# paritytech/reed-solomon-novelpoly

Hardware: AMD Instinct MI355X
Metric: payload GiB/s (device-resident) encode+reconstruct, n=1024 shards, 1 MiB msgs (higher is better)
Workload: dtype u16; 1 GPU; BASELINE config 3: n_wanted=1024 k_wanted=342 (effective n=1024, k=256), 1048576 B payloads, batch 1024/GPU, encode + error locator + reconstruct with 342 random erasures per payload; n=1024, k=256, payload_bytes=1048576, batch_per_gpu=1024, global_batch=1024, erasures=342, parallelism=replicas x1 (no collective)

## Files before the change

### reed-solomon-novelpoly_amd/csrc/fast_common.hpp

```cpp
#pragma once
#include <type_traits>

#include "device_common.hpp"
#include "launchers.hpp"

namespace np {
namespace {

constexpr int kTile = 256;

#ifndef NP_EXP
#define NP_EXP 0
#endif
constexpr int kExp = NP_EXP;

__device__ __forceinline__ void stamp(uint64_t* dbg, int slot) {
  if constexpr ((kExp & 64) != 0 && (kExp & 128) != 0) {
    if ((threadIdx.x & 63u) == 0) dbg[32u * (threadIdx.x >> 6) + slot] = __builtin_amdgcn_s_memtime();
  } else if constexpr (kExp & 64) {
    if (threadIdx.x == 0) dbg[slot] = __builtin_amdgcn_s_memtime();
  }
}
constexpr int kPoolWords = 20;

// ... 955 lines not shown
    x = s;
    y = d;
  } else {
    const int32_t a = static_cast<int32_t>(x), b = static_cast<int32_t>(y);
    x = static_cast<uint32_t>(a + b);
    y = static_cast<uint32_t>(a - b);
  }
}
template <int N, int NT, bool MOD>
__device__ __forceinline__ void lds_wht(uint32_t* W) {
  const uint32_t tid = threadIdx.x;
  int b = 0;
#pragma unroll 1
  for (; (2 << b) < N; b += 2) {
    const uint32_t h = 1u << b;
    for (uint32_t q = tid; q < N / 4; q += NT) {
      const uint32_t i = ((q & ~(h - 1u)) << 2) | (q & (h - 1u));
      uint32_t x0 = W[i], x1 = W[i + h], x2 = W[i + 2 * h], x3 = W[i + 3 * h];
      wht_bfly<MOD>(x0, x1);
      wht_bfly<MOD>(x2, x3);
      wht_bfly<MOD>(x0, x2);
      wht_bfly<MOD>(x1, x3);
      W[i] = x0, W[i + h] = x1, W[i + 2 * h] = x2, W[i + 3 * h] = x3;
    }
    __syncthreads();
  }
  if ((1 << b) < N) {
    const uint32_t h = 1u << b;
    for (uint32_t q = tid; q < N / 2; q += NT) {
      const uint32_t i = ((q & ~(h - 1u)) << 1) | (q & (h - 1u));
      uint32_t x = W[i], y = W[i + h];
      wht_bfly<MOD>(x, y);
      W[i] = x, W[i + h] = y;
    }
    __syncthreads();
  }
}

template <int N, int NT>
__device__ __forceinline__ void fused_locator_core(const DevTables& T, uint32_t* W, uint16_t* E, const uint8_t* PR) {
  const uint32_t tid = threadIdx.x;
  lds_wht<N, NT, false>(W);
  const uint16_t* F = T.lw_fold + N;
  for (uint32_t v = tid; v < N; v += NT) {
    const int32_t x = static_cast<int32_t>(W[v]);
    const uint32_t m = x < 0 ? static_cast<uint32_t>(x + 65535) : static_cast<uint32_t>(x);
    W[v] = (m * static_cast<uint32_t>(F[v])) % 65535u;
  }
  __syncthreads();
  lds_wht<N, NT, true>(W);
  for (uint32_t v = tid; v < N; v += NT) *NP_BCHK(E + v, 2, kBkRecords) = T.exp[NP_ICHK(PR[v] ? W[v] : 65535u - W[v], 65536u)];
}

template <int N, int NT>
__device__ __forceinline__ void fused_locator_pools(const DevTables& T, uint32_t* W, const uint8_t* PR, uint8_t* dst) {
  const uint32_t tid = threadIdx.x;
  lds_wht<N, NT, false>(W);
  const uint16_t* F = T.lw_fold + N;
  for (uint32_t v = tid; v < N; v += NT) {
    const int32_t x = static_cast<int32_t>(W[v]);
    const uint32_t m = x < 0 ? static_cast<uint32_t>(x + 65535) : static_cast<uint32_t>(x);
    W[v] = (m * static_cast<uint32_t>(F[v])) % 65535u;
  }
  __syncthreads();
  lds_wht<N, NT, true>(W);
  for (uint32_t v = tid; v < N; v += NT) {
    const bool p = PR[v] != 0;
    const uint32_t e = T.exp[NP_ICHK(p ? W[v] : 65535u - W[v], 65536u)];
    const uint4* src = reinterpret_cast<const uint4*>((p ? T.in_pools : T.out_pools) + static_cast<size_t>(e) * kPoolWords);
    uint4* d = NP_BCHK(reinterpret_cast<uint4*>(dst + static_cast<size_t>(v) * 4 * kPoolWords), 4 * kPoolWords, kBkRecords);
    const uint4 a0 = src[0], a1 = src[1], a2 = src[2], a3 = src[3], a4 = src[4];
    d[0] = a0, d[1] = a1, d[2] = a2, d[3] = a3, d[4] = a4;
  }
}

template <int N, int NT>
__device__ __forceinline__ void fused_locator(const DevTables& T, const uint8_t* pres, uint32_t* W, uint16_t* E,
                                              uint8_t* PR) {
  const uint32_t tid = threadIdx.x;
  for (uint32_t v = tid; v < N; v += NT) {
    const uint8_t p = *NP_BCHK(pres + v, 1, kBkPresent);
    PR[v] = p;
    W[v] = p ? 0u : 1u;
  }
  __syncthreads();
  fused_locator_core<N, NT>(T, W, E, PR);
}

}
}
```

### reed-solomon-novelpoly_amd/csrc/kernels_fast.hip

```cpp
#include <algorithm>
#include <cstdlib>

#include "fast_common.hpp"

namespace np {
namespace {

constexpr int kEncMaxGen = 3;
__device__ __forceinline__ bool enc_tower(uint32_t index) {
  return __builtin_amdgcn_readfirstlane(gen_of(index)) <= static_cast<uint32_t>(kEncMaxGen);
}

constexpr int kEncPrio = 1, kEncPrioCq = 1;
constexpr int kRecPrioPremul = 2, kRecPrioCq = 3, kRecPrioHi = 2, kRecPrioFwdHi = 3, kRecPrioFwdCq = 2;

template <int K, int SH>
constexpr int kShiftGen = static_cast<int>(gen_of((SH == 23 ? 2 : SH) * K));

template <int K, int SH, typename HOOK = NoHiHook>
__device__ __forceinline__ void shift_hi(const DevTables& T, const uint32_t* vp, uint32_t index,
                                         const uint32_t (&ML)[16], const uint32_t (&MH)[16], uint32_t (&XL)[16],
                                         uint32_t (&XH)[16], uint32_t (&PL)[8], uint32_t (&PH)[8], HOOK hook = HOOK{}) {
#pragma unroll
  for (int q = 0; q < 16; ++q) {
// ... 554 lines not shown
__global__ __launch_bounds__(4 * K) __attribute__((amdgpu_waves_per_eu(4))) void k_encode_multi(EncLaunch L) {
#if defined(__HIP_DEVICE_COMPILE__)
  extern __shared__ __attribute__((aligned(16))) uint8_t smem[];
#if NP_BOUNDS_CHECK
  bounds_arm(bounds_of_enc(L.a));
#endif
  const uint32_t groups = (L.tiles + L.tpw - 1) / L.tpw;
  const TileRef tr = tile_of(blockIdx.x, groups, (L.a.batch & 7u) == 0);
  const uint32_t pb = tr.pb, tl0 = tr.tl * L.tpw;
  const uint32_t ntl = min(L.tpw, L.tiles - tl0);
  const uint64_t kp = reinterpret_cast<uint64_t>(__builtin_amdgcn_kernarg_segment_ptr());
  bool dma = false;
#pragma unroll 1
  for (uint32_t t = 0; t < ntl; ++t) {
    if (t > 0) __syncthreads();
    const enc_launch_ptr lp = reinterpret_cast<enc_launch_ptr>(fresh(kp));
    const DevTables T = lp->T;
    const EncodeArgs a = lp->a;
    const uint32_t pch0 = (tl0 + t - 1) * kTile;
    const bool stored16 = t > 0 && pch0 + kTile <= lp->nchunks &&
                          rows_vec_ok(a.shards, a.batch_stride, a.shard_len) &&
                          (min(a.n / K, (a.wanted_n + K - 1) / K) - 1) * K + 16 * 16 <= a.wanted_n &&
                          16 * a.shard_len < 0x7fffffffu;
    dma = encode_tile_multi<K>(T, a, smem, fresh(pb), fresh(tl0) + t, lp->nchunks, t == 0, dma, stored16,
                               t + 1 < ntl ? tl0 + t + 1 : ~0u);
  }
#endif
}

struct RecCtx {
  const DevTables& T;
  size_t shard_len;
  uint8_t* tile;
  const uint32_t* R;
  const uint8_t* sh;
  uint32_t* VP;
  uint32_t g, lane, tid, ncols;
  bool full;
  uint32_t cqb, hb;
  uint64_t* dbg;
  uint32_t occ;
};

template <int NQ>
__host__ __device__ constexpr int seg_of(int step) {
  return NQ == 8 ? 7 - step : NQ == 4 ? (step == 0 ? 2 : step == 1 ? 3 : 3 - step) : 1 - step;
}

__host__ __device__ constexpr uint32_t rec8_kappa(int q) {
  constexpr uint32_t k[8] = {1, 1, 3, 2, 12, 15, 10, 8};
  return k[q];
}

__device__ __forceinline__ uint32_t row_mask16(const uint8_t* pres, uint32_t row0, uint32_t lane) {
  const bool p = lane < 16u && *NP_BCHK(pres + (row0 + lane), 1, kBkPresent) != 0;
  return static_cast<uint32_t>(__ballot(p));
}

template <int CPOL>
__device__ __forceinline__ void issue_rows_c(uint2 (&raw)[16], const uint8_t* sh, size_t shard_len, uint32_t mask,
                                             uint32_t row0, const uint8_t* zeros, uint32_t lane, uint32_t ncols,
                                             bool full) {
  if (full) {
#pragma unroll
    for (int p = 0; p < 16; ++p) {
      if ((mask >> p) & 1u) NP_BNOTE(sh + static_cast<size_t>(row0 + p) * shard_len + 8u * lane, 8, kBkShards);
      const __amdgpu_buffer_rsrc_t r = buf_rsrc(sh + static_cast<size_t>(row0 + p) * shard_len, ((mask >> p) & 1u) ? 512u : 0u);
      const u32x2 v = __builtin_amdgcn_raw_buffer_load_b64(r, 8u * lane, 0, CPOL);
      raw[p] = make_uint2(v.x, v.y);
    }
  } else {
#pragma unroll
    for (int p = 0; p < 16; ++p) {
      const uint8_t* src = ((mask >> p) & 1u) ? sh + static_cast<size_t>(row0 + p) * shard_len : zeros;
      raw[p] = load4(src, lane, ncols, false);
    }
  }
}

__device__ __forceinline__ void issue_rows(uint2 (&raw)[16], const uint8_t* sh, size_t shard_len, uint32_t mask,
                                           uint32_t row0, const uint8_t* zeros, uint32_t lane, uint32_t ncols,
                                           bool full, bool reread = false) {
  if (!reread)
    issue_rows_c<2>(raw, sh, shard_len, mask, row0, zeros, lane, ncols, full);
  else
    issue_rows_c<0>(raw, sh, shard_len, mask, row0, zeros, lane, ncols, full);
}

template <int K>
__device__ __forceinline__ void copy_out_cq(uint8_t* out_tile, uint32_t lane, uint32_t g, const uint32_t (&L)[16],
                                            const uint32_t (&H)[16]) {
  uint2 d[4][4];
#pragma unroll
  for (int u = 0; u < 4; ++u) cq_to_blks(&L[4 * u], &H[4 * u], d[u]);
#pragma unroll
  for (int i = 0; i < 4; ++i) {
    uint8_t* o = NP_BCHK(out_tile + static_cast<size_t>(4u * lane + i) * 2 * K + 32u * g, 32, kBkOut);
    *reinterpret_cast<uint4*>(o) = make_uint4(d[0][i].x, d[0][i].y, d[1][i].x, d[1][i].y);
    *reinterpret_cast<uint4*>(o + 16) = make_uint4(d[2][i].x, d[2][i].y, d[3][i].x, d[3][i].y);
  }
}


template <int NQ>
constexpr bool kRowPrefetch = NQ <= 2;

template <int K, int NQ>
constexpr bool kRecResident =
    NQ > 1 &&
    Geo<K>::kTileBytes + NQ * 4u * Geo<K>::kVPWords <= 160u * 1024u * Geo<K>::kThreads / 1024u;
template <int K, int NQ>
__device__ __forceinline__ uint32_t vp_slot(int q, int step) {
  return kRecResident<K, NQ> ? static_cast<uint32_t>(q) : static_cast<uint32_t>(step & 1);
}

template <int K, int NQ>
constexpr int kRecMaxGen = static_cast<int>(gen_of(static_cast<uint32_t>((NQ - 1) * K)));

template <int K, int NQ>
__device__ __forceinline__ void stage_rec_tables(const DevTables& T, uint32_t* VP) {
  if constexpr (kRecResident<K, NQ>) {
#pragma unroll 1
    for (int q = 0; q < NQ; ++q)
      stage_vpools<K, Geo<K>::kThreads>(T, static_cast<uint32_t>(q) * K, VP + q * Geo<K>::kVPWords, true);
  } else {
    stage_vpools<K, Geo<K>::kThreads>(T, static_cast<uint32_t>(seg_of<NQ>(0)) * K, VP, true);
    stage_vpools<K, Geo<K>::kThreads>(T, static_cast<uint32_t>(seg_of<NQ>(1)) * K, VP + Geo<K>::kVPWords, true);
  }
}

template <int NQ>
__device__ __forceinline__ uint32_t seg_mask(const uint32_t (&msk)[NQ], int step) {
  if constexpr (NQ <= 2) return step == 0 ? msk[0] : msk[NQ - 1];
  uint64_t lo = 0, hi = 0;
#pragma unroll
  for (int i = 0; i < NQ; ++i) {
    const uint64_t v = static_cast<uint64_t>(msk[i] & 0xffffu);
    if (i < 4)
      lo |= v << (16 * i);
    else
      hi |= v << (16 * (i - 4));
  }
  const uint32_t sh = 16u * static_cast<uint32_t>(step & 3);
  return static_cast<uint32_t>(((step < 4 ? lo : hi) >> sh) & 0xffffu);
}

template <int K, int NQ>
constexpr bool kTilePrefetch = NQ == 4 && kMultiTile<K>;

template <int NQ>
constexpr bool kSkipEmpty = NQ == 8;

template <int K, int NQ, bool PRE0 = false>
__device__ __forceinline__ void rec_segments(const RecCtx& c, const uint32_t (&msk)[NQ], uint2 (&raw)[16],
                                             uint32_t (&AL)[16], uint32_t (&AH)[16], bool after_tile) {
  const DevTables& T = c.T;
  uint32_t XL[16], XH[16];
  auto fold = [&](int step, int q) __attribute__((always_inline)) {
    if (NQ == 8 && q != 0) {
      const uint32_t kq = uniform(rec8_kappa(q));
      if (kq == 1u) {
#pragma unroll
        for (int j = 0; j < 16; ++j) {
          AL[j] ^= XL[j];
          AH[j] ^= XH[j];
        }
      } else {
        uint32_t kp[20];
        pool_of<true>(T, kq, kp);
        const Mult pool = make_mult(kp);
        if (step == 0) {
#pragma unroll
          for (int j = 0; j < 16; ++j) qmul_sub_set(AL[j], AH[j], XL[j], XH[j], pool);
        } else {
#pragma unroll
          for (int j = 0; j < 16; ++j) qmul_sub(AL[j], AH[j], XL[j], XH[j], pool);
        }
      }
    } else if (step == 0) {
#pragma unroll
      for (int j = 0; j < 16; ++j) {
        AL[j] = XL[j];
        AH[j] = XH[j];
      }
    } else if (q == 0) {
      if (NQ == 2 || NQ == 8) {
#pragma unroll
        for (int j = 0; j < 16; ++j) {
          AL[j] ^= XL[j];
          AH[j] ^= XH[j];
        }
      }
      add_derivative<K>(AL, XL, c.tid % Geo<K>::R);
      add_derivative<K>(AH, XH, c.tid % Geo<K>::R);
    } else if (NQ == 4 && q == 3) {
      uint32_t beta[20];
      pool_of<true>(T, 2u, beta);
      const Mult pool = make_mult(beta);
#pragma unroll
      for (int j = 0; j < 16; ++j) {
        XL[j] ^= AL[j];
        XH[j] ^= AH[j];
        qmul_sub(AL[j], AH[j], XL[j], XH[j], pool);
      }
    } else {
#pragma unroll
      for (int j = 0; j < 16; ++j) {
        AL[j] ^= XL[j];
        AH[j] ^= XH[j];
      }
    }
  };
#pragma unroll 1
  for (int step = 0; step < NQ; ++step) {
    const int q = seg_of<NQ>(step);
    if (kSkipEmpty<NQ> && !((c.occ >> q) & 1u)) {
#pragma unroll
      for (int j = 0; j < 16; ++j) XL[j] = XH[j] = 0;
      if constexpr (!kRecResident<K, NQ>) {
        if (step > 0 && step + 1 < NQ) {
          __syncthreads();
          stage_vpools<K, Geo<K>::kThreads>(T, static_cast<uint32_t>(seg_of<NQ>(step + 1)) * K,
                                            c.VP + ((step + 1) & 1) * Geo<K>::kVPWords, true);
          __syncthreads();
        }
      }
    } else {
      const uint32_t index = uniform(static_cast<uint32_t>(q) * K);
      __builtin_amdgcn_sched_barrier(0);
      const uint32_t g = fresh(c.g);
      const uint8_t* sh = fresh(c.sh);
      const uint32_t* R = fresh(c.R);
      const size_t shard_len = fresh(c.shard_len);
      const uint32_t cqb = fresh_v(c.cqb), hb = fresh_v(c.hb);
      uint32_t m = uniform(seg_mask<NQ>(msk, step));
      if (!kRowPrefetch<NQ> && !(PRE0 && step == 0))
        issue_rows(raw, (kExp & 32) ? T.zeros : sh, (kExp & 32) ? 0 : shard_len, m, index + 16 * g, T.zeros, c.lane,
                   c.ncols, c.full, q == 0);
      stamp(c.dbg, 2 + 6 * step);
      __builtin_amdgcn_s_setprio(kRecPrioPremul);
      pipelined_rec<16>(
          [&](auto pc) __attribute__((always_inline)) {
            NP_BNOTE(reinterpret_cast<const uint8_t*>(R) + (index + 16 * g + decltype(pc)::value) * 4 * kPoolWords,
                     4 * kPoolWords, kBkRecords);
            return (cpool_t)(R) + (index + 16 * g + decltype(pc)::value) * kPoolWords;
          },
          [&](auto pc) __attribute__((always_inline)) { return ((m >> decltype(pc)::value) & 1u) != 0; },
          [&](auto pc, const Mult& pool) __attribute__((always_inline)) {
            constexpr int x = decltype(pc)::value;
            XL[x] = 0;
            XH[x] = 0;
            if ((m >> x) & 1u) {
              uint32_t l, h;
              blk_to_quad(raw[x], l, h);
              if constexpr (kExp & 16) {
                XL[x] = l;
                XH[x] = h;
// ... 286 lines not shown
#pragma unroll
          for (int e = 0; e < 8; ++e) o[e] = static_cast<uint8_t>((e < 4 ? v.x : v.y) >> (8 * (e & 3)));
        }
      }
    }
    stamp(dbg, 31);
  }
}

template <int K, int NQ, int SERVE>
__global__ __launch_bounds__(4 * K) __attribute__((amdgpu_waves_per_eu(4))) void k_reconstruct_fast(
    DevTables T, ReconstructArgs a, uint32_t nsyms, uint32_t tiles, uint32_t tpw) {
  constexpr int N = NQ * K;
  extern __shared__ __attribute__((aligned(16))) uint8_t smem[];
#if NP_BOUNDS_CHECK
  bounds_arm(bounds_of(a, T, prefix_stride_c(N, K)));
#endif
  const uint32_t groups = (tiles + tpw - 1) / tpw;
  const TileRef tr = tile_of(blockIdx.x, groups, (a.batch & 7u) == 0);
  const uint32_t pb = tr.pb, tl0 = tr.tl * tpw;
  const uint32_t ntl = min(tpw, tiles - tl0);
  const uint8_t* pres = a.present + static_cast<size_t>(pb) * N;
  const uint8_t* rec = NP_BCHK(a.prefix + static_cast<size_t>(pb) * prefix_stride_c(N, K), 2, kBkRecords);
  const int nq = uniform(rec[0]);
  const uint32_t occ = uniform(rec[1]);
  const uint32_t* rows = reinterpret_cast<const uint32_t*>(rec + prefix_pools_offset(N));
  if constexpr (kMultiTile<K>) {
    if constexpr (SERVE >= 4) {
      if (nq == SERVE) rec_tiles<K, SERVE>(T, a, pres, rows, smem, pb, tl0, ntl, nsyms, occ);
    } else if (nq == 1) {
      rec_tiles<K, 1>(T, a, pres, rows, smem, pb, tl0, ntl, nsyms, occ);
    } else if (NQ <= 4 && nq == 2) {
      rec_tiles<K, 2>(T, a, pres, rows, smem, pb, tl0, ntl, nsyms, occ);
    }
  } else {
    const uint32_t col0 = tl0 * kTile;
    const uint32_t ncols = min(static_cast<uint32_t>(kTile), nsyms - col0);
    const uint8_t* sh = a.shards + static_cast<size_t>(pb) * a.batch_stride + 2 * static_cast<size_t>(col0);
    const bool full =
        ncols == kTile && rows_vec_ok(a.shards, a.batch_stride, a.shard_len);
    uint64_t* dbg = (kExp & 64) ? reinterpret_cast<uint64_t*>(a.out + static_cast<size_t>(pb) * a.out_stride +
                                                               static_cast<size_t>(nsyms) * 2 * K + ((kExp & 128) ? 4096u : 256u) * tl0)
                                 : nullptr;
    if constexpr (SERVE >= 4) {
      if (nq == SERVE) rec_tile<K, SERVE>(T, a, sh, pres, rows, smem, pb, col0, ncols, full, dbg, occ);
    } else if (nq == 1) {
      rec_tile<K, 1>(T, a, sh, pres, rows, smem, pb, col0, ncols, full, dbg, occ);
    } else if (NQ <= 4 && nq == 2) {
      rec_tile<K, 2>(T, a, sh, pres, rows, smem, pb, col0, ncols, full, dbg, occ);
    }
  }
}

__device__ __forceinline__ void write_row_pools(const DevTables& T, const uint16_t* E, const uint8_t* PR,
                                                uint32_t rows, uint8_t* dst) {
  for (uint32_t v = threadIdx.x; v < rows; v += 256) {
    const uint32_t* pools = PR[v] ? T.in_pools : T.out_pools;
    const uint4* src = reinterpret_cast<const uint4*>(pools + static_cast<size_t>(NP_ICHK(*NP_BCHK(E + v, 2, kBkRecords), 65536u)) * kPoolWords);
    uint4* d = NP_BCHK(reinterpret_cast<uint4*>(dst + static_cast<size_t>(v) * 4 * kPoolWords), 4 * kPoolWords, kBkRecords);
    const uint4 a0 = src[0], a1 = src[1], a2 = src[2], a3 = src[3], a4 = src[4];
    d[0] = a0, d[1] = a1, d[2] = a2, d[3] = a3, d[4] = a4;
  }
}


template <int K, int N>
__device__ __forceinline__ void count_present(const uint8_t* pres, int& have1, int& have2, int& have) {
  have1 = have2 = have = 0;
  for (int r = 0; r < N; r += 256) {
    const int v = static_cast<int>(threadIdx.x) + r;
    const bool p = v < N && *NP_BCHK(pres + v, 1, kBkPresent) != 0;
    if (r < K) have1 += __syncthreads_count(v < K && p);
    if (r < 2 * K) have2 += __syncthreads_count(v < 2 * K && p);
    have += __syncthreads_count(p);
  }
}

template <int K, int N>
__device__ __forceinline__ uint32_t segment_occupancy(const uint8_t* pres) {
  uint32_t occ = 0;
#pragma unroll 1
  for (int q = 0; q < N / K; ++q) {
    int any = 0;
    for (int v = static_cast<int>(threadIdx.x); v < K; v += 256) any |= *NP_BCHK(pres + (q * K + v), 1, kBkPresent) != 0;
    if (__syncthreads_or(any)) occ |= 1u << q;
  }
  return occ;
}

__device__ __forceinline__ bool write_status(const ReconstructArgs& a, uint32_t pb, int have) {
  const bool ok = have >= static_cast<int>(a.k);
  if (threadIdx.x == 0 && a.status) {
    *NP_BCHK(a.status + 2 * pb, 4, kBkStatus) = ok ? 0u : kStatusNeedMoreShards;
    *NP_BCHK(a.status + 2 * pb + 1, 4, kBkStatus) = static_cast<uint32_t>(have);
  }
  return ok;
}

template <int N>
constexpr int kPrefixThreads = N >= 512 ? 512 : 256;

template <int K, int NQ, int NT = kPrefixThreads<NQ * K>>
__global__ __launch_bounds__(NT) void k_prefix_locator(DevTables T, ReconstructArgs a, uint8_t* out) {
  constexpr int N = NQ * K;
  __shared__ uint32_t W[N];
  __shared__ uint8_t PR[N];
  const uint32_t pb = blockIdx.x, tid = threadIdx.x;
#if NP_BOUNDS_CHECK
  {
    ReconstructArgs ab = a;
    ab.prefix = out;
    bounds_arm(bounds_of(ab, T, prefix_stride_c(N, K)));
  }
#endif
  const uint8_t* pres = a.present + static_cast<size_t>(pb) * N;
  uint8_t* rec = out + static_cast<size_t>(pb) * prefix_stride_c(N, K);
  __shared__ uint32_t acc[4];
  if (tid < 4) acc[tid] = 0;
  __syncthreads();
  {
    uint32_t c1 = 0, c2 = 0, c = 0, occ = 0;
    for (uint32_t v = tid; v < static_cast<uint32_t>(N); v += NT) {
      const uint8_t p = *NP_BCHK(pres + v, 1, kBkPresent);
      PR[v] = p;
      W[v] = p ? 0u : 1u;
      const uint32_t on = p ? 1u : 0u;
      c += on;
      c1 += v < static_cast<uint32_t>(K) ? on : 0u;
      c2 += v < 2u * K ? on : 0u;
      occ |= on << (v / K);
    }
#pragma unroll
    for (int o = 32; o > 0; o >>= 1) {
      c1 += __shfl_xor(c1, o);
      c2 += __shfl_xor(c2, o);
      c += __shfl_xor(c, o);
      occ |= __shfl_xor(occ, o);
    }
    if ((tid & 63u) == 0) {
      atomicAdd(&acc[0], c1);
      atomicAdd(&acc[1], c2);
      atomicAdd(&acc[2], c);
      atomicOr(&acc[3], occ);
    }
  }
  __syncthreads();
  const int have1 = static_cast<int>(acc[0]), have2 = static_cast<int>(acc[1]), have = static_cast<int>(acc[2]);
  const int nq = !write_status(a, pb, have) ? 0 : have1 == K ? 1 : (a.trusted && NQ == 4 && have2 >= K) ? 2 : NQ;
  if (tid == 0) *NP_BCHK(rec, 2, kBkRecords) = static_cast<uint8_t>(nq), *NP_BCHK(rec + 1, 1, kBkRecords) = static_cast<uint8_t>(acc[3]);
  if (nq <= 1) return;
  if (NQ == 4 && nq == 2) {
    fused_locator_pools<2 * K, NT>(T, W, PR, rec + prefix_pools_offset(N));
  } else {
    fused_locator_pools<N, NT>(T, W, PR, rec + prefix_pools_offset(N));
  }
}

template <int K, int NQ>
__global__ __launch_bounds__(256) void k_locator_records(DevTables T, ReconstructArgs a, uint8_t* out) {
  constexpr int N = NQ * K;
  const uint32_t pb = blockIdx.x, tid = threadIdx.x;
#if NP_BOUNDS_CHECK
  {
    ReconstructArgs ab = a;
    ab.prefix = out;
    bounds_arm(bounds_of(ab, T, prefix_stride_c(N, K)));
  }
#endif
  const uint16_t* loc = a.locators + static_cast<size_t>(pb) * N;
  uint8_t* rec = out + static_cast<size_t>(pb) * prefix_stride_c(N, K);
  uint16_t* E = reinterpret_cast<uint16_t*>(rec + kPrefixHeader);
  int have1, have2, have;
  count_present<K, N>(a.present + static_cast<size_t>(pb) * N, have1, have2, have);
  const bool ok = write_status(a, pb, have);
  const uint32_t occ = segment_occupancy<K, N>(a.present + static_cast<size_t>(pb) * N);
  if (tid == 0) *NP_BCHK(rec, 2, kBkRecords) = static_cast<uint8_t>(ok ? NQ : 0), *NP_BCHK(rec + 1, 1, kBkRecords) = static_cast<uint8_t>(occ);
  if (!ok) return;
  for (uint32_t v = tid; v < static_cast<uint32_t>(N); v += 256) *NP_BCHK(E + v, 2, kBkRecords) = T.exp[*NP_BCHK(loc + v, 2, kBkLocators)];
  write_row_pools(T, E, a.present + static_cast<size_t>(pb) * N, N, rec + prefix_pools_offset(N));
}

template <int K>
size_t encode_lds_bytes() {
  return static_cast<size_t>(Geo<K>::kTileBytes) + 4u * 4u * Geo<K>::kVPWords;
}

template <int K>
size_t encode_multi_lds_bytes() {
  return static_cast<size_t>(Geo<K>::kTileBytes) + kEncBuffers * 4u * Geo<K>::kVPWords;
}


template <int K, int NQ>
size_t reconstruct_lds_bytes() {
  return static_cast<size_t>(Geo<K>::kTileBytes) + (kRecResident<K, NQ> ? NQ : 2) * 4u * Geo<K>::kVPWords;
}

constexpr size_t kWorkgroups = 1024;

template <int K>
uint32_t tiles_per_workgroup(size_t batch, uint32_t tiles, const char* knob) {
  if (!kMultiTile<K>) return 1;
  size_t want = batch * tiles / kWorkgroups;
  if (const char* e = std::getenv(knob)) want = std::strtoul(e, nullptr, 10);
  return static_cast<uint32_t>(std::max<size_t>(1, std::min<size_t>(tiles, want)));
}

template <typename TPW, typename F>
hipError_t with_encode_grid(const EncodeArgs& a, TPW tpw_of, F launch) {
  const size_t nchunks = (a.payload_len + 2 * a.k - 1) / (2 * a.k);
  if (nchunks == 0 || a.batch == 0) return hipSuccess;
  if (nchunks > 0xffffffffu) return hipErrorInvalidValue;
  const uint32_t tiles = static_cast<uint32_t>((nchunks + kTile - 1) / kTile);
  const uint32_t tpw = tpw_of(tiles);
  const size_t blocks = a.batch * ((tiles + tpw - 1) / tpw);
  if (blocks > 0x7fffffffu) return hipErrorInvalidValue;
  launch(static_cast<uint32_t>(nchunks), tiles, tpw, static_cast<uint32_t>(blocks));
  return hipGetLastError();
}
uint32_t one_tile(uint32_t) { return 1u; }

template <int K>
hipError_t launch_encode_k(const DevTables& T, const EncodeArgs& a, hipStream_t s) {
  const bool multi = kMultiTile<K> && a.n <= kEncBuffers * K;
  return with_encode_grid(
      a, [&](uint32_t tiles) { return multi ? tiles_per_workgroup<K>(a.batch, tiles, "NP_ENC_TPW") : 1u; },
      [&](uint32_t nchunks, uint32_t tiles, uint32_t tpw, uint32_t blocks) {
        if constexpr (kMultiTile<K>) {
          if (multi) {
            k_encode_multi<K><<<blocks, Geo<K>::kThreads, encode_multi_lds_bytes<K>(), s>>>(
                EncLaunch{T, a, nchunks, tiles, tpw});
            return;
// ... 594 lines not shown
```

### reed-solomon-novelpoly_amd/csrc/kernels_res.hip

```cpp
#include "res_common.hpp"

namespace np {
namespace {

constexpr int kResPrioEnc = 1, kResPrioDec = 1, kResPrioDecCq = 1;

template <int K>
__global__ __launch_bounds__(K) __attribute__((amdgpu_waves_per_eu(4))) void k_encode_res(
    DevTables T, EncodeArgs a, uint32_t nchunks, uint32_t tiles) {
  extern __shared__ __attribute__((aligned(16))) uint8_t smem[];
  uint8_t* tile = smem;
#if NP_BOUNDS_CHECK
  bounds_arm(bounds_of_enc(a));
#endif
  const TileRef tr = tile_of(blockIdx.x, tiles, (a.batch & 7u) == 0);
  const uint32_t pb = tr.pb, tl = tr.tl;
  const uint32_t ch0 = tl * kRC;
  const uint32_t ncols = min(static_cast<uint32_t>(kRC), nchunks - ch0);
  const uint8_t* pay = a.payloads + static_cast<size_t>(pb) * a.payload_stride;
  uint8_t* out = a.shards + static_cast<size_t>(pb) * a.batch_stride + 2 * static_cast<size_t>(ch0);
  const Res r = res_coords<K>();
  const Qi qc = qi_coords<K>(r);
  const bool full =
      ncols == kRC && rows_vec_ok(a.shards, a.batch_stride, a.shard_len);
// ... 133 lines not shown
  }
  rstamp(dbg, s0 + 2);
  __syncthreads();
  rcq_write<K>(tile, fresh_v(rr.cqb), XL, XH);
  __syncthreads();
  rh_read<kHA>(tile, fresh_v(rr.hab), XL, XH);
  rstamp(dbg, s0 + 3);
  const uint32_t* vs = DL + kDeltaWords + q * RStage<K>::kWords;
  if constexpr (kResNoHD<K>) {
    if constexpr (STEP + 1 < NQ) {
      __syncthreads();
      dma_row_tables(tile, pools, static_cast<uint32_t>(res_seg<NQ>(STEP + 1)) * K, K, rr.w, rr.l, K / 64);
    }
    ha_levels_st<K, true, res_gen<K>(I), kResPrioDec>(T, I, rr, XL, XH, vs);
    rstamp(dbg, s0 + 4);
    if constexpr (q == 0) {
      __syncthreads();
      rh_write<kHA>(tile, fresh_v(rr.hab), XL, XH);
      __syncthreads();
      rh_read<kHD>(tile, fresh_v(rr.hdb), XL, XH);
      uint32_t YL[16], YH[16];
#pragma unroll
      for (int j = 0; j < 16; ++j) {
        YL[j] = (NQ == 2 || NQ == 8) ? XL[j] : 0u;
        YH[j] = (NQ == 2 || NQ == 8) ? XH[j] : 0u;
      }
      add_derivative_hd<K>(YL, XL, rr.l);
      add_derivative_hd<K>(YH, XH, rr.l);
      __syncthreads();
      rh_write<kHD>(tile, fresh_v(rr.hdb), YL, YH);
      __syncthreads();
      rh_read<kHA>(tile, fresh_v(rr.hab), YL, YH);
#pragma unroll
      for (int j = 0; j < 16; ++j) AL[j] ^= YL[j], AH[j] ^= YH[j];
      rstamp(dbg, s0 + 7);
      return true;
    }
  } else {
  ha_levels_st<K, true, res_gen<K>(I), kResPrioDec>(T, I, rr, XL, XH, vs);
  rstamp(dbg, s0 + 4);
  __syncthreads();
  rh_write<kHA>(tile, fresh_v(rr.hab), XL, XH);
  __syncthreads();
  rh_read<kHD>(tile, fresh_v(rr.hdb), XL, XH);
  if constexpr (STEP + 1 < NQ) {
    __syncthreads();
    dma_row_tables(tile, pools, static_cast<uint32_t>(res_seg<NQ>(STEP + 1)) * K, K, rr.w, rr.l, K / 64);
  }
  rstamp(dbg, s0 + 5);
  hd_levels_st<K, true, kResPrioDec>(T, I, XL, XH, vs);
  rstamp(dbg, s0 + 6);
  }
  }
  if constexpr (NQ == 8 && q != 0 && rec8_kappa_res(q) != 1u) {
    uint32_t kp[20];
    pool_of<true>(T, rec8_kappa_res(q), kp);
    const Mult m = make_mult(kp);
#pragma unroll
    for (int j = 0; j < 16; ++j) {
      if constexpr (STEP == 0)
        qmul_sub_set(AL[j], AH[j], XL[j], XH[j], m);
      else
        qmul_sub(AL[j], AH[j], XL[j], XH[j], m);
    }
  } else if constexpr (STEP == 0) {
#pragma unroll
    for (int j = 0; j < 16; ++j) AL[j] = XL[j], AH[j] = XH[j];
  } else if constexpr (q == 0) {
    if constexpr (NQ == 2 || NQ == 8) {
#pragma unroll
      for (int j = 0; j < 16; ++j) AL[j] ^= XL[j], AH[j] ^= XH[j];
    }
    add_derivative_hd<K>(AL, XL, rr.l);
    add_derivative_hd<K>(AH, XH, rr.l);
  } else if constexpr (NQ == 4 && q == 3) {
    uint32_t beta[20];
    pool_of<true>(T, 2u, beta);
    const Mult m = make_mult(beta);
#pragma unroll
    for (int j = 0; j < 16; ++j) {
      XL[j] ^= AL[j];
      XH[j] ^= AH[j];
      qmul_sub(AL[j], AH[j], XL[j], XH[j], m);
    }
  } else {
#pragma unroll
    for (int j = 0; j < 16; ++j) AL[j] ^= XL[j], AH[j] ^= XH[j];
  }
  rstamp(dbg, s0 + 7);
  return true;
}

template <int K, int NQ, int... STEP>
__device__ __forceinline__ bool res_sweep(const DevTables& T, const ReconstructArgs& a, uint8_t* tile,
                                          const uint8_t* pools, const uint8_t* pres, const uint8_t* sh,
                                          uint8_t* out_tile, uint32_t ncols, bool full, bool out16,
                                          uint32_t (&AL)[16], uint32_t (&AH)[16], uint64_t* dbg, uint32_t occ,
                                          std::integer_sequence<int, STEP...>) {
  return (res_step<K, NQ, STEP>(T, a, tile, pools, pres, sh, out_tile, ncols, full, out16, AL, AH, dbg, occ) && ...);
}

template <int K, int NQ>
__device__ __forceinline__ void res_decode_tile(const DevTables& T, const ReconstructArgs& a, uint8_t* tile,
                                                const uint8_t* pools, const uint8_t* pres, const uint8_t* sh,
                                                uint8_t* out_tile, uint32_t ncols, bool full, bool out16,
                                                uint64_t* dbg, uint32_t occ) {
  uint32_t AL[16], AH[16];
  uint32_t* DL = reinterpret_cast<uint32_t*>(tile + RGeo<K>::kTileBytes);
  uint32_t* VS = DL + kDeltaWords;
  rstamp(dbg, 0);
  {
    const Res r0 = res_coords<K>();
    dma_row_tables(tile, pools, static_cast<uint32_t>(res_seg<NQ>(0)) * K, K, r0.w, r0.l, K / 64);
  }
  stage_delta_tables(T, DL);
  stage_rh_tables<K>(T, VS, NQ);
  rstamp(dbg, 1);
  if (!res_sweep<K, NQ>(T, a, tile, pools, pres, sh, out_tile, ncols, full, out16, AL, AH, dbg, occ,
                     std::make_integer_sequence<int, NQ>{}))
    return;
  constexpr uint32_t kHD = RGeo<K>::kHD, lpc = RGeo<K>::kLPC;
  const Res r = res_coords<K>();
  if constexpr ((kExp & 8192) != 0 && !kResNoHD<K>) {
    const uint32_t c = (64u / lpc) * r.w + r.l / lpc;
#pragma unroll
    for (int j = 0; j < 16; ++j)
      if (c < ncols)
        *reinterpret_cast<uint2*>(out_tile + static_cast<size_t>(c) * 2 * K + 8u * (r.l % lpc + lpc * j)) =
            quad_to_blk(AL[j], AH[j]);
    return;
  }
  if constexpr (!kResNoHD<K>) {
    hd_levels_st<K, false, kResPrioDec>(T, 0, AL, AH, VS);
    rstamp(dbg, 40);
    __syncthreads();
    rh_write<kHD>(tile, fresh_v(r.hdb), AL, AH);
    __syncthreads();
    rh_read<kHA>(tile, fresh_v(r.hab), AL, AH);
  }
  rstamp(dbg, 41);
  ha_levels_st<K, false, 0, kResPrioDec>(T, 0, r, AL, AH, VS);
// ... 173 lines not shown
```

### reed-solomon-novelpoly_amd/csrc/kernels_small.hip

```cpp
#include "fast_common.hpp"

namespace np {
namespace {

constexpr int kSmallMaxSeg = 8;

__device__ __forceinline__ uint32_t lo(uint64_t q) { return static_cast<uint32_t>(q); }
__device__ __forceinline__ uint32_t hi(uint64_t q) { return static_cast<uint32_t>(q >> 32); }
__device__ __forceinline__ uint64_t quad(uint32_t l, uint32_t h) { return (static_cast<uint64_t>(h) << 32) | l; }

__device__ __forceinline__ void qmul_q(uint64_t& x, uint64_t y, const Mult& m) {
  uint32_t xl = lo(x), xh = hi(x);
  qmul_sub(xl, xh, lo(y), hi(y), m);
  x = quad(xl, xh);
}

template <int K, bool INVERSE>
__host__ __device__ constexpr GroupRef reg_group(int f) {
  constexpr int lg = ilog2(K);
  for (int s = 0; s < lg; ++s) {
    const int b = INVERSE ? s : lg - 1 - s, n = K >> (b + 1);
    if (f < n) return GroupRef{b, f};
    f -= n;
  }
// ... 191 lines not shown
        for (int i = 0; i < 4; ++i) {
          const u32x4 v = __builtin_nontemporal_load(reinterpret_cast<const u32x4*>(pay + c0 + i * 2 * K + 16 * u2));
          d0[i] = make_uint2(v.x, v.y);
          d1[i] = make_uint2(v.z, v.w);
        }
        blks_to_q(d0, &M[8 * u2]);
        blks_to_q(d1, &M[8 * u2 + 4]);
      }
    } else {
      constexpr int kBlk = K < 4 ? 1 : K / 4, kBytes = K < 4 ? 2 * K : 8;
#pragma unroll
      for (int u = 0; u < kBlk; ++u) {
        uint2 d[4];
#pragma unroll
        for (int i = 0; i < 4; ++i) {
          const size_t g0 = c0 + static_cast<size_t>(i) * 2 * K + 8u * u;
          uint32_t w[2] = {0, 0};
#pragma unroll
          for (int e = 0; e < kBytes; ++e)
            if (g0 + e < a.payload_len) w[e >> 2] |= static_cast<uint32_t>(pay[g0 + e]) << (8 * (e & 3));
          d[i] = make_uint2(w[0], w[1]);
        }
        if constexpr (K >= 4) {
          blks_to_q(d, &M[4 * u]);
        } else {
          uint64_t Q4[4];
          blks_to_q(d, Q4);
#pragma unroll
          for (int p = 0; p < K; ++p) M[p] = Q4[p];
        }
      }
    }
  }
  store_rows_k<K>(out, a.shard_len, 0, a.wanted_n, M, lane, ncols, full, rows_nt(a.shards, a.batch_stride, a.shard_len));
  tower_convert_q(T, M);
  reg_levels<K, true, true>(T, VP, 0, M);
#pragma unroll
  for (int p = 0; p < K; ++p) asm volatile("" : "+v"(M[p]));

#pragma unroll 1
  for (uint32_t s = 1; s < nshift && s * K < a.wanted_n; ++s) {
    const uint32_t index = uniform(s * K);
    const uint32_t live = a.wanted_n - index;
    const uint32_t rows = live >= static_cast<uint32_t>(K) ? ~0u : (1u << live) - 1u;
    uint64_t X[K];
#pragma unroll
    for (int p = 0; p < K; ++p) X[p] = M[p];
    reg_levels<K, false, false>(T, VP + s * G::kVPWords, index, X, uniform(rows));
    tower_convert_q(T, X);
    store_rows_k<K>(out, a.shard_len, index, a.wanted_n, X, lane, ncols, full, rows_nt(a.shards, a.batch_stride, a.shard_len));
  }
}

__device__ __forceinline__ uint32_t small_kappa(int nq, int q) {
  if (nq == 2) return 1u;
  if (nq == 4) return q == 0 ? 0u : q == 1 ? 1u : q == 2 ? 3u : 2u;
  return q < 2 ? 1u : q == 2 ? 3u : q == 3 ? 2u : q == 4 ? 12u : q == 5 ? 15u : q == 6 ? 10u : 8u;
}

template <int K, int NQ>
__global__ __launch_bounds__(256) void k_reconstruct_small(DevTables T, ReconstructArgs a, uint32_t nsyms,
                                                           uint32_t tiles) {
  using G = Geo<K>;
  constexpr int N = NQ * K;
#if NP_BOUNDS_CHECK
  bounds_arm(bounds_of(a, T, prefix_stride_c(N, K)));
#endif
  __shared__ __attribute__((aligned(16))) uint32_t VP[NQ * G::kVPWords];
  for (int q = 0; q < NQ; ++q) stage_vpools<K, 256>(T, static_cast<uint32_t>(q) * K, VP + q * G::kVPWords, true);
  __syncthreads();
  uint32_t pb, tl;
  if (!wave_tile(a.batch, tiles, pb, tl)) return;
  const uint8_t* rec = a.prefix + static_cast<size_t>(pb) * prefix_stride_c(N, K);
  const int nq = uniform(rec[0]);
  if (nq == 0) return;
  const uint32_t* R = reinterpret_cast<const uint32_t*>(rec + prefix_pools_offset(N));
  const uint8_t* pres = a.present + static_cast<size_t>(pb) * N;
  const uint32_t lane = threadIdx.x & 63u;
  const uint32_t col0 = tl * kTile;
  const uint32_t ncols = min(static_cast<uint32_t>(kTile), nsyms - col0);
  const uint8_t* sh = a.shards + static_cast<size_t>(pb) * a.batch_stride + 2 * static_cast<size_t>(col0);
  const bool full =
      ncols == kTile && rows_vec_ok(a.shards, a.batch_stride, a.shard_len);
  const uint32_t m0 = uniform(static_cast<uint32_t>(__ballot(lane < K && pres[lane] != 0)));

  uint64_t X[K];
  if (nq == 1) {
    uint2 raw[K];
    load_rows_k<K, 2>(raw, sh, a.shard_len, m0, 0, T.zeros, lane, ncols, full);
#pragma unroll
    for (int p = 0; p < K; ++p) X[p] = blk_quad(raw[p]);
  } else {
    uint64_t A[K];
#pragma unroll
    for (int p = 0; p < K; ++p) A[p] = 0;
#pragma unroll 1
    for (int q = nq - 1; q >= 0; --q) {
      const uint32_t row0 = uniform(static_cast<uint32_t>(q) * K);
      const uint32_t m = q == 0 ? m0 : uniform(static_cast<uint32_t>(__ballot(lane < K && pres[row0 + lane] != 0)));
      if (m == 0) continue;
      {
        uint2 raw[K];
        if (q == 0)
          load_rows_k<K, 0>(raw, sh, a.shard_len, m, 0, T.zeros, lane, ncols, full);
        else
          load_rows_k<K, 2>(raw, sh, a.shard_len, m, row0, T.zeros, lane, ncols, full);
        pipelined_rec<K>(
            [&](auto pc) __attribute__((always_inline)) { return (cpool_t)(R) + (row0 + decltype(pc)::value) * kPoolWords; },
            [&](auto pc) __attribute__((always_inline)) { return ((m >> decltype(pc)::value) & 1u) != 0; },
            [&](auto pc, const Mult& pool) __attribute__((always_inline)) {
              constexpr int x = decltype(pc)::value;
              X[x] = 0;
              if ((m >> x) & 1u) {
                uint32_t l, h, xl, xh;
                blk_to_quad(raw[x], l, h);
                qmul_set(xl, xh, l, h, pool);
                X[x] = quad(xl, xh);
              }
            });
      }
      const uint32_t* vp = VP + q * G::kVPWords;
      if (q == 0) {
        reg_levels<K, true, true>(T, vp, 0, X, m);
        add_derivative_reg<K>(A, X);
      } else {
        reg_levels<K, true, false>(T, vp, row0, X, m);
      }
      const uint32_t kq = uniform(small_kappa(nq, q));
      if (kq == 1u) {
#pragma unroll
        for (int p = 0; p < K; ++p) A[p] ^= X[p];
      } else if (kq != 0u) {
        uint32_t kp[20];
        pool_of<true>(T, kq, kp);
        const Mult pool = make_mult(kp);
#pragma unroll
        for (int p = 0; p < K; ++p) qmul_q(A[p], X[p], pool);
      }
    }
    reg_levels<K, false, true>(T, VP, 0, A, ~m0);
    uint2 raw[K];
    load_rows_k<K, 2>(raw, sh, a.shard_len, m0, 0, T.zeros, lane, ncols, full);
    pipelined_rec<K>(
        [&](auto pc) __attribute__((always_inline)) { return (cpool_t)(R) + decltype(pc)::value * kPoolWords; },
        [&](auto pc) __attribute__((always_inline)) { return ((m0 >> decltype(pc)::value) & 1u) == 0; },
        [&](auto pc, const Mult& pool) __attribute__((always_inline)) {
          constexpr int x = decltype(pc)::value;
          if ((m0 >> x) & 1u) {
            X[x] = blk_quad(raw[x]);
          } else {
            uint32_t xl, xh;
            qmul_set(xl, xh, lo(A[x]), hi(A[x]), pool);
            X[x] = quad(xl, xh);
          }
        });
  }
  uint8_t* out = a.out + static_cast<size_t>(pb) * a.out_stride + static_cast<size_t>(col0) * 2 * K;
  const bool al16 = full && out_vec_ok(a.out, a.out_stride);
  const bool al8 = true;
  if constexpr (K < 8) {
    uint64_t Q4[4] = {0, 0, 0, 0};
#pragma unroll
    for (int p = 0; p < K; ++p) Q4[p] = X[p];
    uint2 d[4];
    q_to_blks(Q4, d);
#pragma unroll
    for (int i = 0; i < 4; ++i) {
      const uint32_t c = 4u * lane + i;
      uint8_t* o = out + static_cast<size_t>(c) * 2 * K;
      if (c < ncols) {
        if constexpr (K == 4) {
          if (al8) {
            *reinterpret_cast<uint2*>(o) = d[i];
          } else {
#pragma unroll
            for (int e = 0; e < 8; ++e) o[e] = static_cast<uint8_t>((e < 4 ? d[i].x : d[i].y) >> (8 * (e & 3)));
          }
        } else {
#pragma unroll
          for (int e = 0; e < 2 * K; ++e) o[e] = static_cast<uint8_t>(d[i].x >> (8 * e));
        }
      }
    }
    return;
  }
#pragma unroll
  for (int u2 = 0; u2 < K / 8; ++u2) {
    uint2 d0[4], d1[4];
    q_to_blks(&X[8 * u2], d0);
    q_to_blks(&X[8 * u2 + 4], d1);
// ... 91 lines not shown
```

Before: 245.5 GiB/s.

## Fold per-segment kappa scaling into locator pool records instead of reconstruct

Per-segment kappa constants used to be applied in the reconstruct inner loops as extra GF multiplies on the accumulated quad vectors. They are now folded into the per-row multiplier pools at locator time, by adding log(kappa) to each present row's log before the exp lookup. The reconstruct fold then reduces to plain XOR, removing the per-segment multiplies and pool loads from the hot loop. Scheduling barriers are added around the fold in the resident kernel. This relies on the algebraic identity holding for every NQ path, including the special NQ==4 q==3 case that used a different combining formula.

```diff
diff --git a/reed-solomon-novelpoly_amd/csrc/fast_common.hpp b/reed-solomon-novelpoly_amd/csrc/fast_common.hpp
--- a/reed-solomon-novelpoly_amd/csrc/fast_common.hpp
+++ b/reed-solomon-novelpoly_amd/csrc/fast_common.hpp
@@ -1031,8 +1031,15 @@
   for (uint32_t v = tid; v < N; v += NT) *NP_BCHK(E + v, 2, kBkRecords) = T.exp[NP_ICHK(PR[v] ? W[v] : 65535u - W[v], 65536u)];
 }
 
-template <int N, int NT>
-__device__ __forceinline__ void fused_locator_pools(const DevTables& T, uint32_t* W, const uint8_t* PR, uint8_t* dst) {
+__device__ __forceinline__ uint32_t scaled_log(uint32_t x, uint32_t l) {
+  if (l == 0u) return x;
+  x += l;
+  return x >= 65535u ? x - 65535u : x;
+}
+
+template <int N, int NT, int KSEG = 0>
+__device__ __forceinline__ void fused_locator_pools(const DevTables& T, uint32_t* W, const uint8_t* PR, uint8_t* dst,
+                                                    const uint32_t* lk = nullptr) {
   const uint32_t tid = threadIdx.x;
   lds_wht<N, NT, false>(W);
   const uint16_t* F = T.lw_fold + N;
@@ -1045,7 +1052,9 @@
   lds_wht<N, NT, true>(W);
   for (uint32_t v = tid; v < N; v += NT) {
     const bool p = PR[v] != 0;
-    const uint32_t e = T.exp[NP_ICHK(p ? W[v] : 65535u - W[v], 65536u)];
+    uint32_t x = p ? W[v] : 65535u - W[v];
+    if constexpr (KSEG != 0) x = p ? scaled_log(x, lk[v / KSEG]) : x;
+    const uint32_t e = T.exp[NP_ICHK(x, 65536u)];
     const uint4* src = reinterpret_cast<const uint4*>((p ? T.in_pools : T.out_pools) + static_cast<size_t>(e) * kPoolWords);
     uint4* d = NP_BCHK(reinterpret_cast<uint4*>(dst + static_cast<size_t>(v) * 4 * kPoolWords), 4 * kPoolWords, kBkRecords);
     const uint4 a0 = src[0], a1 = src[1], a2 = src[2], a3 = src[3], a4 = src[4];
diff --git a/reed-solomon-novelpoly_amd/csrc/kernels_fast.hip b/reed-solomon-novelpoly_amd/csrc/kernels_fast.hip
--- a/reed-solomon-novelpoly_amd/csrc/kernels_fast.hip
+++ b/reed-solomon-novelpoly_amd/csrc/kernels_fast.hip
@@ -630,6 +630,19 @@
   return k[q];
 }
 
+template <int NQ>
+__host__ __device__ constexpr uint32_t seg_kappa(int q) {
+  return q == 0 ? 1u : NQ == 8 ? rec8_kappa(q) : NQ == 4 ? (q == 2 ? 3u : q == 3 ? 2u : 1u) : 1u;
+}
+
+template <int NQ>
+__device__ __forceinline__ void stage_seg_logs(const DevTables& T, uint32_t* lk) {
+  if (threadIdx.x < static_cast<uint32_t>(NQ)) {
+    const uint32_t kq = seg_kappa<NQ>(static_cast<int>(threadIdx.x));
+    lk[threadIdx.x] = kq == 1u ? 0u : T.log[kq];
+  }
+}
+
 __device__ __forceinline__ uint32_t row_mask16(const uint8_t* pres, uint32_t row0, uint32_t lane) {
   const bool p = lane < 16u && *NP_BCHK(pres + (row0 + lane), 1, kBkPresent) != 0;
   return static_cast<uint32_t>(__ballot(p));
@@ -735,27 +748,7 @@
   const DevTables& T = c.T;
   uint32_t XL[16], XH[16];
   auto fold = [&](int step, int q) __attribute__((always_inline)) {
-    if (NQ == 8 && q != 0) {
-      const uint32_t kq = uniform(rec8_kappa(q));
-      if (kq == 1u) {
-#pragma unroll
-        for (int j = 0; j < 16; ++j) {
-          AL[j] ^= XL[j];
-          AH[j] ^= XH[j];
-        }
-      } else {
-        uint32_t kp[20];
-        pool_of<true>(T, kq, kp);
-        const Mult pool = make_mult(kp);
-        if (step == 0) {
-#pragma unroll
-          for (int j = 0; j < 16; ++j) qmul_sub_set(AL[j], AH[j], XL[j], XH[j], pool);
-        } else {
-#pragma unroll
-          for (int j = 0; j < 16; ++j) qmul_sub(AL[j], AH[j], XL[j], XH[j], pool);
-        }
-      }
-    } else if (step == 0) {
+    if (step == 0) {
 #pragma unroll
       for (int j = 0; j < 16; ++j) {
         AL[j] = XL[j];
@@ -771,16 +764,6 @@
       }
       add_derivative<K>(AL, XL, c.tid % Geo<K>::R);
       add_derivative<K>(AH, XH, c.tid % Geo<K>::R);
-    } else if (NQ == 4 && q == 3) {
-      uint32_t beta[20];
-      pool_of<true>(T, 2u, beta);
-      const Mult pool = make_mult(beta);
-#pragma unroll
-      for (int j = 0; j < 16; ++j) {
-        XL[j] ^= AL[j];
-        XH[j] ^= AH[j];
-        qmul_sub(AL[j], AH[j], XL[j], XH[j], pool);
-      }
     } else {
 #pragma unroll
       for (int j = 0; j < 16; ++j) {
@@ -1173,11 +1156,15 @@
   }
 }
 
+template <int KSEG>
 __device__ __forceinline__ void write_row_pools(const DevTables& T, const uint16_t* E, const uint8_t* PR,
-                                                uint32_t rows, uint8_t* dst) {
+                                                uint32_t rows, uint8_t* dst, const uint16_t* loc, const uint32_t* lk) {
   for (uint32_t v = threadIdx.x; v < rows; v += 256) {
     const uint32_t* pools = PR[v] ? T.in_pools : T.out_pools;
-    const uint4* src = reinterpret_cast<const uint4*>(pools + static_cast<size_t>(NP_ICHK(*NP_BCHK(E + v, 2, kBkRecords), 65536u)) * kPoolWords);
+    uint32_t e = NP_ICHK(*NP_BCHK(E + v, 2, kBkRecords), 65536u);
+    const uint32_t l = lk[v / KSEG];
+    if (PR[v] && l != 0u) e = T.exp[scaled_log(*NP_BCHK(loc + v, 2, kBkLocators), l)];
+    const uint4* src = reinterpret_cast<const uint4*>(pools + static_cast<size_t>(e) * kPoolWords);
     uint4* d = NP_BCHK(reinterpret_cast<uint4*>(dst + static_cast<size_t>(v) * 4 * kPoolWords), 4 * kPoolWords, kBkRecords);
     const uint4 a0 = src[0], a1 = src[1], a2 = src[2], a3 = src[3], a4 = src[4];
     d[0] = a0, d[1] = a1, d[2] = a2, d[3] = a3, d[4] = a4;
@@ -1237,7 +1224,9 @@
   const uint8_t* pres = a.present + static_cast<size_t>(pb) * N;
   uint8_t* rec = out + static_cast<size_t>(pb) * prefix_stride_c(N, K);
   __shared__ uint32_t acc[4];
+  __shared__ uint32_t LK[NQ];
   if (tid < 4) acc[tid] = 0;
+  stage_seg_logs<NQ>(T, LK);
   __syncthreads();
   {
     uint32_t c1 = 0, c2 = 0, c = 0, occ = 0;
@@ -1273,7 +1262,7 @@
   if (NQ == 4 && nq == 2) {
     fused_locator_pools<2 * K, NT>(T, W, PR, rec + prefix_pools_offset(N));
   } else {
-    fused_locator_pools<N, NT>(T, W, PR, rec + prefix_pools_offset(N));
+    fused_locator_pools<N, NT, (NQ > 2 ? K : 0)>(T, W, PR, rec + prefix_pools_offset(N), LK);
   }
 }
 
@@ -1291,6 +1280,8 @@
   const uint16_t* loc = a.locators + static_cast<size_t>(pb) * N;
   uint8_t* rec = out + static_cast<size_t>(pb) * prefix_stride_c(N, K);
   uint16_t* E = reinterpret_cast<uint16_t*>(rec + kPrefixHeader);
+  __shared__ uint32_t LK[NQ];
+  stage_seg_logs<NQ>(T, LK);
   int have1, have2, have;
   count_present<K, N>(a.present + static_cast<size_t>(pb) * N, have1, have2, have);
   const bool ok = write_status(a, pb, have);
@@ -1298,7 +1289,7 @@
   if (tid == 0) *NP_BCHK(rec, 2, kBkRecords) = static_cast<uint8_t>(ok ? NQ : 0), *NP_BCHK(rec + 1, 1, kBkRecords) = static_cast<uint8_t>(occ);
   if (!ok) return;
   for (uint32_t v = tid; v < static_cast<uint32_t>(N); v += 256) *NP_BCHK(E + v, 2, kBkRecords) = T.exp[*NP_BCHK(loc + v, 2, kBkLocators)];
-  write_row_pools(T, E, a.present + static_cast<size_t>(pb) * N, N, rec + prefix_pools_offset(N));
+  write_row_pools<K>(T, E, a.present + static_cast<size_t>(pb) * N, N, rec + prefix_pools_offset(N), loc, LK);
 }
 
 template <int K>
diff --git a/reed-solomon-novelpoly_amd/csrc/kernels_res.hip b/reed-solomon-novelpoly_amd/csrc/kernels_res.hip
--- a/reed-solomon-novelpoly_amd/csrc/kernels_res.hip
+++ b/reed-solomon-novelpoly_amd/csrc/kernels_res.hip
@@ -209,18 +209,10 @@
   rstamp(dbg, s0 + 6);
   }
   }
-  if constexpr (NQ == 8 && q != 0 && rec8_kappa_res(q) != 1u) {
-    uint32_t kp[20];
-    pool_of<true>(T, rec8_kappa_res(q), kp);
-    const Mult m = make_mult(kp);
-#pragma unroll
-    for (int j = 0; j < 16; ++j) {
-      if constexpr (STEP == 0)
-        qmul_sub_set(AL[j], AH[j], XL[j], XH[j], m);
-      else
-        qmul_sub(AL[j], AH[j], XL[j], XH[j], m);
-    }
-  } else if constexpr (STEP == 0) {
+  __builtin_amdgcn_sched_barrier(0);
+#pragma unroll
+  for (int j = 0; j < 16; ++j) asm volatile("" : "+v"(XL[j]), "+v"(XH[j]));
+  if constexpr (STEP == 0) {
 #pragma unroll
     for (int j = 0; j < 16; ++j) AL[j] = XL[j], AH[j] = XH[j];
   } else if constexpr (q == 0) {
@@ -230,20 +222,13 @@
     }
     add_derivative_hd<K>(AL, XL, rr.l);
     add_derivative_hd<K>(AH, XH, rr.l);
-  } else if constexpr (NQ == 4 && q == 3) {
-    uint32_t beta[20];
-    pool_of<true>(T, 2u, beta);
-    const Mult m = make_mult(beta);
-#pragma unroll
-    for (int j = 0; j < 16; ++j) {
-      XL[j] ^= AL[j];
-      XH[j] ^= AH[j];
-      qmul_sub(AL[j], AH[j], XL[j], XH[j], m);
-    }
   } else {
 #pragma unroll
     for (int j = 0; j < 16; ++j) AL[j] ^= XL[j], AH[j] ^= XH[j];
   }
+#pragma unroll
+  for (int j = 0; j < 16; ++j) asm volatile("" : "+v"(AL[j]), "+v"(AH[j]));
+  __builtin_amdgcn_sched_barrier(0);
   rstamp(dbg, s0 + 7);
   return true;
 }
diff --git a/reed-solomon-novelpoly_amd/csrc/kernels_small.hip b/reed-solomon-novelpoly_amd/csrc/kernels_small.hip
--- a/reed-solomon-novelpoly_amd/csrc/kernels_small.hip
+++ b/reed-solomon-novelpoly_amd/csrc/kernels_small.hip
@@ -267,11 +267,7 @@
   }
 }
 
-__device__ __forceinline__ uint32_t small_kappa(int nq, int q) {
-  if (nq == 2) return 1u;
-  if (nq == 4) return q == 0 ? 0u : q == 1 ? 1u : q == 2 ? 3u : 2u;
-  return q < 2 ? 1u : q == 2 ? 3u : q == 3 ? 2u : q == 4 ? 12u : q == 5 ? 15u : q == 6 ? 10u : 8u;
-}
+__device__ __forceinline__ bool small_folds(int nq, int q) { return q != 0 || nq != 4; }
 
 template <int K, int NQ>
 __global__ __launch_bounds__(256) void k_reconstruct_small(DevTables T, ReconstructArgs a, uint32_t nsyms,
@@ -341,16 +337,9 @@
       } else {
         reg_levels<K, true, false>(T, vp, row0, X, m);
       }
-      const uint32_t kq = uniform(small_kappa(nq, q));
-      if (kq == 1u) {
+      if (small_folds(nq, q)) {
 #pragma unroll
         for (int p = 0; p < K; ++p) A[p] ^= X[p];
-      } else if (kq != 0u) {
-        uint32_t kp[20];
-        pool_of<true>(T, kq, kp);
-        const Mult pool = make_mult(kp);
-#pragma unroll
-        for (int p = 0; p < K; ++p) qmul_q(A[p], X[p], pool);
       }
     }
     reg_levels<K, false, true>(T, VP, 0, A, ~m0);
```

After: 245.3 GiB/s. No clear change (-0.1%).
